# dmlc/difacto

Hardware: AMD Instinct MI355X
Metric: examples/sec (FM SGD worker step, Criteo-shape, V_dim=64) (higher is better)
Workload: dtype f32

## Files before the change

### difacto_amd/csrc/dfh_api.hip

```cpp
#include <algorithm>
#include <chrono>
#include <cstring>
#include <mutex>
#include <new>
#include <thread>

#include <hip/hip_ext.h>
#include <rocprim/rocprim.hpp>

#include "dfh_kernels.hip"
#include "dfh_localize.hip"
#include "dfh_update.hip"
#include "dfh_riders.hip"

using namespace dfh;

namespace dfh {
static thread_local std::string g_err;
void set_error(const std::string& msg) { g_err = msg; }
}

struct dfh_ctx {
  int device = 0;
  hipStream_t stream = nullptr;
// ... 33 lines not shown
  std::vector<hipEvent_t> pool;
  double t_ms[DFH_K_COUNT] = {0};
  uint64_t t_calls[DFH_K_COUNT] = {0};
};

namespace {
struct TimeScope {
  dfh_ctx* c;
  int id;
  hipStream_t st;
  hipEvent_t a = nullptr, b = nullptr;
  static hipEvent_t get(dfh_ctx* c) {
    if (!c->pool.empty()) {
      hipEvent_t e = c->pool.back();
      c->pool.pop_back();
      return e;
    }
    hipEvent_t e = nullptr;
    if (hipEventCreate(&e) != hipSuccess) return nullptr;
    return e;
  }
  TimeScope(dfh_ctx* ctx, int kid, hipStream_t s = nullptr) : c(ctx), id(kid), st(s ? s : ctx->stream) {
    if (kid >= DFH_K_COUNT || !((c->timing >> kid) & 1u)) return;
    a = get(c);
    b = get(c);
    if (a && b) (void)hipEventRecord(a, st);
  }
  ~TimeScope() {
    if (!a || !b) return;
    (void)hipEventRecord(b, st);
    c->spans.push_back({id, a, b});
  }
};
}

struct dfh_table {
  dfh_ctx* ctx = nullptr;
  TableView v{};
  uint64_t hslots = 0;
  uint64_t bytes = 0;
  bool has_aux = true;
  bool auto_grow = false;
  uint64_t rows_bound = 0;
  uint64_t grows = 0;
  uint32_t* d_need = nullptr;
  uint32_t* d_rank = nullptr;
  uint32_t* d_urow = nullptr;
  uint32_t* d_total = nullptr;
  size_t aux_cap = 0;
};

struct dfh_batch {
  dfh_ctx* ctx = nullptr;
  size_t max_rows = 0, max_nnz = 0;
  size_t nrows = 0, nnz = 0;
  bool has_value = false;
  bool has_cnt = false;
  bool localized = false;
  uint64_t* d_raw = nullptr;
  uint32_t* d_offset = nullptr;
  float* d_value = nullptr;
  float* d_label = nullptr;
  void* arena = nullptr;
  void* shared_arena = nullptr;
  size_t arena_bytes = 0;
  uint64_t* o_raw = nullptr;
  uint32_t* o_offset = nullptr;
  float* o_value = nullptr;
  float* o_label = nullptr;
  char* h_stage = nullptr;
  size_t stage_bytes = 0;
  hipEvent_t ev_staged = nullptr;
  bool staged_pending = false;
  double t_prof[6] = {0, 0, 0, 0, 0, 0};
  uint64_t n_prof = 0;
  char* d_stage_view = nullptr;
  bool defer_ready = false;
  uint64_t *d_keys = nullptr, *d_skeys = nullptr;
  uint32_t *d_pos = nullptr, *d_spos = nullptr;
  uint32_t *d_bpos = nullptr;
  uint32_t *d_head = nullptr, *d_uid = nullptr;
  void* d_temp = nullptr;
  size_t temp_bytes = 0;
  uint64_t *d_smp_key = nullptr, *d_spl_key = nullptr, *d_first_key = nullptr, *d_last_key = nullptr;
  uint32_t *d_smp_rank = nullptr, *d_smp_pos = nullptr, *d_spl_pos = nullptr, *d_packed = nullptr, *d_run_off = nullptr,
           *d_bstart = nullptr, *d_btotal = nullptr, *d_nheads = nullptr, *d_lh = nullptr;
  size_t max_tiles = 0;
  int spl_P = 0;
  uint64_t* d_feaids = nullptr;
  float* d_feacnt = nullptr;
  uint32_t *d_col_ptr = nullptr, *d_index = nullptr, *d_s_row = nullptr;
  float* d_s_val = nullptr;
  uint32_t* d_U = nullptr;
  uint2 *d_mid = nullptr, *d_hot = nullptr, *d_few = nullptr;
  SegEnt *d_mid_ent = nullptr, *d_hot_ent = nullptr, *d_few_ent = nullptr;
  SegEnt* d_split_ent = nullptr;
  uint32_t* d_split_ticket = nullptr;
  float* d_split_part = nullptr;
  size_t split_cap = 0;
  int split_sel = 0, split_last = 0;
  bool split_listing = false;
  uint32_t seg_nb = 0;
  uint2* d_uw = nullptr;
  uint32_t *d_urow = nullptr, *d_need = nullptr, *d_rank = nullptr, *d_total = nullptr;
  float *d_pred = nullptr, *d_slope = nullptr, *d_xv = nullptr;
  size_t xv_floats = 0;
  double* d_prog = nullptr;
  float nrows_seen = 0;
  hipEvent_t ev_ready = nullptr, ev_free = nullptr;
  bool ready_pending = false, free_pending = false;
  hipStream_t prep = nullptr;
  bool compute_auc = false;
  uint32_t *d_auc_keys = nullptr, *d_auc_skeys = nullptr, *d_auc_lab = nullptr, *d_auc_slab = nullptr;
  uint32_t* d_auc_part = nullptr;
  uint32_t auc_pending_n = 0;
  bool force_radix = false;
  bool force_sort_fallback = false;
  dfh_table* looked_up = nullptr;
  struct GatherSeg { struct dfh_rowbuf* rb; size_t at, n; };
  std::vector<GatherSeg> gsegs;
  GatherSrc gsrc{};
  bool gather_pending = false, gather_fusable = false, gather_any_value = false, loc_fuse_gather = false;
  const uint32_t *g_rows = nullptr, *g_off = nullptr;
  const float* g_lab = nullptr;
  LocView loc_v{};
  EmitOut loc_o{};
  uint32_t loc_gsort = 0;
  bool loc_big = false;
  int pend_stage = RID_STAGES;
};

namespace {
int flush_pending(dfh_batch* b);
void pend_remove(dfh_ctx* c, dfh_batch* b);
inline hipStream_t prep_of(const dfh_batch* b) {
  const dfh_ctx* c = b->ctx;
  return (c->pipeline && b->prep) ? b->prep : c->stream;
}
void phase_begin(dfh_batch* b) {
  dfh_ctx* c = b->ctx;
  if (b->pend_stage < RID_STAGES) (void)flush_pending(b);
  hipStream_t next = c->pipeline ? c->preps[c->next_prep++ % c->nprep] : nullptr;
  if (next && b->prep && next != b->prep && b->ready_pending) {
    (void)hipStreamWaitEvent(next, b->ev_ready, 0);
  }
  b->prep = next;
}
int prep_begin(dfh_batch* b) {
  dfh_ctx* c = b->ctx;
  if (c->pipeline && !b->prep) phase_begin(b);
  if (c->pipeline && b->free_pending) {
    DFH_HIP(hipStreamWaitEvent(prep_of(b), b->ev_free, 0));
    b->free_pending = false;
  }
  return DFH_OK;
}
int prep_end(dfh_batch* b) {
  dfh_ctx* c = b->ctx;
  if (c->pipeline && !b->defer_ready) {
    DFH_HIP(hipEventRecord(b->ev_ready, prep_of(b)));
    b->ready_pending = true;
  }
  return DFH_OK;
}
int main_begin(dfh_batch* b) {
  dfh_ctx* c = b->ctx;
  if (b->pend_stage < RID_STAGES) {
    int rc = flush_pending(b);
    if (rc) return rc;
// ... 1773 lines not shown
namespace {
struct SharedArena {
  void* base = nullptr;
  int refs = 0;
};
}

static int batch_create_impl(dfh_ctx* c, size_t max_rows, size_t max_nnz, dfh_batch** out, SharedArena* shared, size_t at,
                             size_t* size_only, bool sync) {
  DFH_ARG(c && (out || size_only) && max_rows >= 1 && max_nnz >= 1, "dfh_batch_create: bad argument");
  DFH_ARG(max_nnz < 0xFFFFFFF0ULL && max_rows < 0xFFFFFFF0ULL, "batch too large for 32-bit positions");
  DFH_HIP(hipSetDevice(c->device));
  dfh_batch* b = new (std::nothrow) dfh_batch();
  DFH_ARG(b != nullptr, "out of host memory");
  b->ctx = c;
  b->max_rows = max_rows;
  b->max_nnz = max_nnz;
  const size_t N = max_nnz, B = max_rows;
  size_t sort_bytes = 0, scan_bytes = 0;
  rocprim::radix_sort_pairs(nullptr, sort_bytes, (uint64_t*)nullptr, (uint64_t*)nullptr, (uint32_t*)nullptr,
                            (uint32_t*)nullptr, N, 0, 64, c->stream);
  rocprim::inclusive_scan(nullptr, scan_bytes, (uint32_t*)nullptr, (uint32_t*)nullptr, N, rocprim::plus<uint32_t>(), c->stream);
  size_t auc_bytes = 0;
  rocprim::radix_sort_pairs(nullptr, auc_bytes, (uint32_t*)nullptr, (uint32_t*)nullptr, (uint32_t*)nullptr,
                            (uint32_t*)nullptr, B, 0, 32, c->stream);
  b->temp_bytes = std::max(std::max(sort_bytes, scan_bytes), auc_bytes) + 256;
  char* arena_at = nullptr;
  size_t arena_need = 0;
  bool sizing = true;
#define DFH_ALLOC(ptr, count, type)                                                        \
  do {                                                                                     \
    const size_t bytes__ = (((size_t)(count) * sizeof(type)) + 255) & ~(size_t)255;        \
    if (sizing) {                                                                          \
      arena_need += bytes__;                                                               \
    } else {                                                                               \
      (ptr) = reinterpret_cast<type*>(arena_at);                                           \
      arena_at += bytes__;                                                                 \
    }                                                                                      \
  } while (0)
  for (int pass = 0; pass < 2; ++pass) {
  sizing = pass == 0;
  if (!sizing) {
    if (size_only) {
      *size_only = arena_need;
      delete b;
      return DFH_OK;
    }
    if (shared) {
      b->shared_arena = shared;
      ++shared->refs;
      arena_at = static_cast<char*>(shared->base) + at;
    } else {
      hipError_t e__ = hipMalloc(reinterpret_cast<void**>(&b->arena), arena_need);
      if (e__ != hipSuccess) {
        set_error(std::string("dfh_batch_create: hipMalloc: ") + hipGetErrorString(e__));
        dfh_batch_destroy(b);
        return DFH_ERR_HIP;
      }
      arena_at = static_cast<char*>(b->arena);
    }
  }
  DFH_ALLOC(b->o_raw, N, uint64_t);
  DFH_ALLOC(b->o_offset, B + 1, uint32_t);
  DFH_ALLOC(b->o_value, N, float);
  DFH_ALLOC(b->o_label, B, float);
  b->d_raw = b->o_raw;
  b->d_offset = b->o_offset;
  b->d_value = b->o_value;
  b->d_label = b->o_label;
  DFH_ALLOC(b->d_keys, N, uint64_t);
  DFH_ALLOC(b->d_skeys, N, uint64_t);
  DFH_ALLOC(b->d_pos, N, uint32_t);
  DFH_ALLOC(b->d_spos, N, uint32_t);
  DFH_ALLOC(b->d_bpos, N, uint32_t);
  DFH_ALLOC(b->d_head, N, uint32_t);
  DFH_ALLOC(b->d_uid, N, uint32_t);
  DFH_ALLOC(b->d_temp, b->temp_bytes, char);
  b->max_tiles = (N + LOC_TILE - 1) / LOC_TILE;
  DFH_ALLOC(b->d_spl_key, LOC_BIG_BUCKETS, uint64_t);
  DFH_ALLOC(b->d_spl_pos, LOC_BIG_BUCKETS, uint32_t);
  DFH_ALLOC(b->d_smp_key, LOC_BIG_BUCKETS * LOC_OVERSAMPLE, uint64_t);
  DFH_ALLOC(b->d_smp_pos, LOC_BIG_BUCKETS * LOC_OVERSAMPLE, uint32_t);
  DFH_ALLOC(b->d_smp_rank, LOC_BIG_BUCKETS * LOC_OVERSAMPLE, uint32_t);
  DFH_ALLOC(b->d_first_key, LOC_BIG_BUCKETS, uint64_t);
  DFH_ALLOC(b->d_last_key, LOC_BIG_BUCKETS, uint64_t);
  DFH_ALLOC(b->d_packed, N, uint32_t);
  DFH_ALLOC(b->d_run_off, b->max_tiles * LOC_BIG_BUCKETS, uint32_t);
  DFH_ALLOC(b->d_bstart, LOC_BIG_BUCKETS + 1, uint32_t);
  DFH_ALLOC(b->d_btotal, LOC_XCDS * LOC_BIG_BUCKETS, uint32_t);
  DFH_ALLOC(b->d_nheads, LOC_BIG_BUCKETS, uint32_t);
  DFH_ALLOC(b->d_lh, LOC_BIG_BUCKETS, uint32_t);
  DFH_ALLOC(b->d_feaids, N, uint64_t);
  DFH_ALLOC(b->d_feacnt, N, float);
  DFH_ALLOC(b->d_col_ptr, N + 1, uint32_t);
  DFH_ALLOC(b->d_index, N, uint32_t);
  DFH_ALLOC(b->d_s_row, N, uint32_t);
  DFH_ALLOC(b->d_s_val, N, float);
  DFH_ALLOC(b->d_U, 64, uint32_t);
  DFH_ALLOC(b->d_urow, N, uint32_t);
  DFH_ALLOC(b->d_uw, N, uint2);
  DFH_ALLOC(b->d_mid_ent, N / (BWD_SMALL + 1) + 2 * LOC_BIG_BUCKETS + 16, SegEnt);
  DFH_ALLOC(b->d_hot_ent, N / (BWD_MID + 1) + 2 * LOC_BIG_BUCKETS + 16, SegEnt);
  DFH_ALLOC(b->d_few_ent, N / 2 + 2 * LOC_BIG_BUCKETS + 16, SegEnt);
  b->split_cap = 2 * (N / HOT_SPLIT) + 16;
  DFH_ALLOC(b->d_split_ent, b->split_cap, SegEnt);
  DFH_ALLOC(b->d_split_ticket, b->split_cap, uint32_t);
  DFH_ALLOC(b->d_split_part, b->split_cap * UPD_SPLIT_STRIDE, float);
  DFH_ALLOC(b->d_mid, LOC_BIG_BUCKETS, uint2);
  DFH_ALLOC(b->d_hot, LOC_BIG_BUCKETS, uint2);
  DFH_ALLOC(b->d_few, LOC_BIG_BUCKETS, uint2);
  DFH_ALLOC(b->d_need, N, uint32_t);
  DFH_ALLOC(b->d_rank, N, uint32_t);
  DFH_ALLOC(b->d_pred, B, float);
  DFH_ALLOC(b->d_slope, B, float);
  DFH_ALLOC(b->d_prog, 2 * PROG_SLOTS + 64, double);
  DFH_ALLOC(b->d_auc_keys, B, uint32_t);
  DFH_ALLOC(b->d_auc_skeys, B, uint32_t);
  DFH_ALLOC(b->d_auc_lab, B, uint32_t);
  DFH_ALLOC(b->d_auc_slab, B, uint32_t);
  DFH_ALLOC(b->d_auc_part, AUC_PART_WORDS, uint32_t);
  }
#undef DFH_ALLOC
  b->arena_bytes = arena_need;
  b->d_total = b->d_U + 1;
  const unsigned evf = hipEventDisableTiming | (c->event_flags ? hipEventDisableSystemFence : 0u);
  hipError_t e2 = hipEventCreateWithFlags(&b->ev_ready, evf);
  if (e2 == hipSuccess) e2 = hipEventCreateWithFlags(&b->ev_free, evf);
  if (e2 == hipSuccess) e2 = hipMemsetAsync(b->d_prog, 0, (2 * PROG_SLOTS + 64) * sizeof(double), c->stream);
  if (e2 == hipSuccess) e2 = hipMemsetAsync(b->d_U, 0, 64 * sizeof(uint32_t), c->stream);
  if (e2 == hipSuccess) e2 = hipMemsetAsync(b->d_split_ticket, 0, b->split_cap * sizeof(uint32_t), c->stream);
  if (e2 == hipSuccess) e2 = hipMemsetAsync(b->d_btotal, 0, LOC_XCDS * LOC_BIG_BUCKETS * sizeof(uint32_t), c->stream);
  if (e2 == hipSuccess) e2 = hipMemsetAsync(b->d_urow, 0xFF, N * sizeof(uint32_t), c->stream);
  if (e2 == hipSuccess) e2 = hipMemsetAsync(b->d_uw, 0xFF, N * sizeof(uint2), c->stream);
  if (e2 == hipSuccess && sync) e2 = hipStreamSynchronize(c->stream);
  if (e2 != hipSuccess) {
    set_error(std::string("dfh_batch_create: ") + hipGetErrorString(e2));
    dfh_batch_destroy(b);
    return DFH_ERR_HIP;
  }
  *out = b;
  return DFH_OK;
}

int dfh_batch_create(dfh_ctx* c, size_t max_rows, size_t max_nnz, dfh_batch** out) {
  return batch_create_impl(c, max_rows, max_nnz, out, nullptr, 0, nullptr, true);
}

int dfh_batch_create_many(dfh_ctx* c, int n, size_t max_rows, size_t max_nnz, dfh_batch** out) {
  DFH_ARG(c && out && n >= 1 && n <= 64, "dfh_batch_create_many: 1 <= n <= 64 objects");
  size_t each = 0;
  int rc = batch_create_impl(c, max_rows, max_nnz, nullptr, nullptr, 0, &each, false);
  if (rc) return rc;
  each = (each + 4095) & ~(size_t)4095;
  SharedArena* sa = new (std::nothrow) SharedArena();
  DFH_ARG(sa != nullptr, "out of host memory");
  DFH_HIP(hipSetDevice(c->device));
  if (hipMalloc(&sa->base, each * (size_t)n) != hipSuccess) {
    delete sa;
    set_error("dfh_batch_create_many: hipMalloc failed");
    return DFH_ERR_HIP;
  }
  for (int i = 0; i < n; ++i) out[i] = nullptr;
  sa->refs = 1;
  for (int i = 0; i < n && !rc; ++i) rc = batch_create_impl(c, max_rows, max_nnz, &out[i], sa, each * (size_t)i, nullptr, false);
  if (!rc && hipStreamSynchronize(c->stream) != hipSuccess) {
    set_error("dfh_batch_create_many: hipStreamSynchronize failed");
    rc = DFH_ERR_HIP;
  }
  if (rc) {
    for (int j = 0; j < n; ++j) {
      if (out[j]) dfh_batch_destroy(out[j]);
      out[j] = nullptr;
    }
  }
// ... 583 lines not shown
    rs->period = std::max(1u, per);
  }
}

int localize_impl(dfh_batch* b, uint64_t max_index, dfh_table* probe) {
  dfh_ctx* c = b->ctx;
  DFH_HIP(hipSetDevice(c->device));
  const uint32_t N = (uint32_t)b->nnz;
  if (probe && N) {
    if (int rcr = table_reserve(probe, N)) return rcr;
  }
  {
    int rc = prep_begin(b);
    if (rc) return rc;
  }
  hipStream_t s = prep_of(b);
  b->looked_up = nullptr;
  if (b->pend_stage < RID_STAGES) {
    int rc = flush_pending(b);
    if (rc) return rc;
  }
  if (N == 0) {
    if (b->gather_pending) {
      int rcg = gather_alone(b, s);
      if (rcg) return rcg;
    }
    DFH_HIP(hipMemsetAsync(b->d_U, 0, 64 * sizeof(uint32_t), s));
    DFH_HIP(hipMemsetAsync(b->d_col_ptr, 0, 4, s));
    b->seg_nb = 0;
    b->localized = true;
    return prep_end(b);
  }
  const int g = grid_for_threads(N, c);
  TimeScope* tsp = new TimeScope(c, DFH_K_LOCALIZE, s);
  int P = 0;
  bool cold = true;
  if (b->spl_P > 0 && N / (uint32_t)b->spl_P >= (uint32_t)LOC_MIN_AVG && N / (uint32_t)b->spl_P <= (uint32_t)LOC_MAX_AVG) {
    P = b->spl_P;
    cold = false;
  } else {
#ifndef DFH_LOC_SMALL_AVG
#define DFH_LOC_SMALL_AVG 192
#endif
    const size_t avg_bucket = N <= 65536u ? (size_t)DFH_LOC_SMALL_AVG : (size_t)LOC_AVG_BUCKET;
    const size_t P_want = (N + avg_bucket - 1) / avg_bucket;
    if (P_want <= (size_t)LOC_MAX_BUCKETS) P = (int)std::max<size_t>(1, P_want);
    else if (N / LOC_MAX_BUCKETS <= (uint32_t)LOC_MAX_AVG) P = LOC_MAX_BUCKETS;
    else if (P_want <= (size_t)LOC_BIG_BUCKETS) P = (int)P_want;
    else if (N / LOC_BIG_BUCKETS <= (uint32_t)LOC_MAX_AVG) P = LOC_BIG_BUCKETS;
  }
  b->loc_fuse_gather = b->gather_pending && b->gather_fusable && !cold && P > 0 && P <= LOC_MAX_BUCKETS && !b->force_radix &&
                       !c->single_queue && !getenv("DFH_GATHER_ALONE");
  if (b->gather_pending && !b->loc_fuse_gather) {
    int rcg = gather_alone(b, s);
    if (rcg) return rcg;
  }
  if (P > 0 && !b->force_radix) {
    LocView& v = b->loc_v;
    v.raw = b->d_raw;
    v.n = N;
    v.max_index = max_index;
    v.P = P;
    const bool big = P > LOC_MAX_BUCKETS;
    v.bstride = big ? LOC_BIG_BUCKETS : LOC_MAX_BUCKETS;
    v.ntiles = (int)((N + LOC_TILE - 1) / LOC_TILE);
    v.force_global = b->force_sort_fallback ? 1 : 0;
    v.tb = N > 1 ? std::min(16, __builtin_clz(N - 1)) : 16;
    v.nrows = (uint32_t)b->nrows;
    v.offset = b->d_offset;
    v.rowid = b->d_pos;
    v.smp_key = b->d_smp_key;
    v.smp_pos = b->d_smp_pos;
    v.smp_rank = b->d_smp_rank;
    v.spl_key = b->d_spl_key;
    v.spl_pos = b->d_spl_pos;
    v.packed = b->d_packed;
    v.run_off = b->d_run_off;
    v.btotal = b->d_btotal;
    v.bstart = b->d_bstart;
    v.bkeys = b->d_keys;
    v.bpos = b->d_bpos;
    v.skeys = b->d_skeys;
    v.spos = b->d_spos;
    v.first_key = b->d_first_key;
    v.last_key = b->d_last_key;
    v.nheads = b->d_nheads;
    v.lh = b->d_lh;
    EmitOut& o = b->loc_o;
    o.value = b->has_value ? b->d_value : (const float*)nullptr;
    o.feaids = b->d_feaids;
    o.col_ptr = b->d_col_ptr;
    o.index = b->d_index;
    o.s_row = b->d_s_row;
    o.s_val = b->d_s_val;
    o.d_U = b->d_U;
    o.sl.mid = b->d_mid;
    o.sl.mid_ent = b->d_mid_ent;
    o.sl.hot = b->d_hot;
    o.sl.hot_ent = b->d_hot_ent;
    o.sl.few = b->d_few;
    o.sl.few_ent = b->d_few_ent;
    v.split_n = b->d_U + 2;
    b->loc_big = big;
#ifndef DFH_LOC_GRID_CAP
#define DFH_LOC_GRID_CAP 1024
#endif
    b->loc_gsort = (unsigned)std::min<int>(P, big ? LOC_BIG_BUCKETS : DFH_LOC_GRID_CAP);
    if (cold && P > 1) {
      const uint32_t S = (uint32_t)P * LOC_OVERSAMPLE;
      const uint32_t nt = (S + 255) / 256;
      hipLaunchKernelGGL(k_ss_sample, dim3(nt), dim3(256), 0, s, v);
      hipLaunchKernelGGL(k_ss_rank, dim3(nt * nt), dim3(256), 0, s, v);
      hipLaunchKernelGGL(k_loc_splitters, dim3(nt), dim3(256), 0, s, v);
    }
    if (c->single_queue && !cold && !big && !probe) {
      b->pend_stage = 0;
      c->pend.push_back(b);
    } else {
      for (int st = 0; st < RID_STAGES; ++st) {
        launch_loc_stage(b, st, s, probe);
        if (st == RID_COUNT && b->loc_fuse_gather) {
          int rcg = gather_queued(b, s);
          b->loc_fuse_gather = false;
          if (rcg) return rcg;
        }
      }
    }
    b->spl_P = P;
    b->seg_nb = (uint32_t)P;
  } else {
    hipLaunchKernelGGL(k_rdx_keys, dim3(g), dim3(256), 0, s, b->d_raw, N, max_index, b->d_keys, b->d_pos);
    size_t tb = b->temp_bytes;
    DFH_HIP(rocprim::radix_sort_pairs(b->d_temp, tb, b->d_keys, b->d_skeys, b->d_pos, b->d_spos, (size_t)N, 0, 64, s));
    hipLaunchKernelGGL(k_rdx_heads, dim3(g), dim3(256), 0, s, b->d_skeys, N, b->d_head);
    tb = b->temp_bytes;
    DFH_HIP(rocprim::inclusive_scan(b->d_temp, tb, b->d_head, b->d_uid, (size_t)N, rocprim::plus<uint32_t>(), s));
    hipLaunchKernelGGL(k_rdx_emit, dim3(g), dim3(256), 0, s, b->d_skeys, b->d_spos, b->d_head, b->d_uid, N, (uint32_t)b->nrows,
                       b->d_offset, b->has_value ? b->d_value : (const float*)nullptr, b->d_feaids, b->d_col_ptr, b->d_index,
                       b->d_s_row, b->d_s_val, b->d_U);
    hipLaunchKernelGGL(k_seg_lists_reset, dim3(1), dim3(64), 0, s, b->d_mid, b->d_hot, b->d_few, b->d_U + 2);
    hipLaunchKernelGGL(k_seg_lists, dim3((unsigned)std::max<size_t>(1, std::min<size_t>((N + 1023) / 1024, 256))), dim3(1024), 0, s,
                       b->d_col_ptr, b->d_U, b->d_mid, b->d_hot, b->d_few, b->d_mid_ent, b->d_hot_ent, b->d_few_ent);
    b->seg_nb = 1;
    if (probe)
      hipLaunchKernelGGL(k_lookup, dim3(grid_for_threads(b->nnz, c)), dim3(256), 0, s, probe->v, b->d_feaids, b->d_U, 0u, b->d_urow,
                         (const float*)nullptr, b->d_col_ptr, 0, (uint32_t*)nullptr, 0, (uint2*)nullptr, AucFin{nullptr, 0u, nullptr});
  }
  delete tsp;
  DFH_HIP(hipGetLastError());
  b->localized = true;
  b->has_cnt = false;
  if (probe) b->looked_up = probe;
  return prep_end(b);
}
}


namespace {
struct DescribedIn {
  size_t nrows, nnz;
  int nseg;
  dfh_rowbuf* const* bufs;
  const size_t* seg_rows;
  bool any_value;
  const uint32_t *v_rows, *v_off;
  const float* v_lab;
  const uint32_t* v_tile;
  bool fusable;
  const uint32_t* v_base;
};
// ... 656 lines not shown
```

### difacto_amd/csrc/dfh_localize.hip

```cpp
#ifndef DFH_LOCALIZE_HIP_
#define DFH_LOCALIZE_HIP_
#include "dfh_internal.h"

namespace dfh {

constexpr int LOC_OVERSAMPLE = 8;
constexpr int LOC_MAX_BUCKETS = 1024;
constexpr int LOC_BIG_BUCKETS = 4096;
constexpr int LOC_AVG_BUCKET = 384;
constexpr int LOC_MIN_AVG = 48;
constexpr int LOC_MAX_AVG = 700;
constexpr int LOC_LDS_CAP = 1024;
#ifndef DFH_LOC_TILE
#define DFH_LOC_TILE 2048
#endif
#ifndef DFH_LOC_TILE_THREADS
#define DFH_LOC_TILE_THREADS 1024
#endif
constexpr int LOC_TILE = DFH_LOC_TILE;
constexpr int LOC_TILE_THREADS = DFH_LOC_TILE_THREADS;
constexpr int LOC_PER_THREAD = LOC_TILE / LOC_TILE_THREADS;
constexpr int LOC_SORT_THREADS = 256;
constexpr int LOC_EMIT_THREADS = 256;

struct LocView {
  const uint64_t* raw;
  uint32_t n;
  uint64_t max_index;
  int P;
  int bstride;
  int ntiles;
  int force_global;
  int tb;
  uint32_t nrows;
  const uint32_t* offset;
  const uint32_t* rowid;
  uint64_t* smp_key;
  uint32_t* smp_pos;
  uint32_t* smp_rank;
  uint64_t* spl_key;
  uint32_t* spl_pos;
  uint32_t* packed;
  uint32_t* run_off;
  uint32_t* btotal;
  uint32_t* bstart;
  uint64_t* bkeys;
  uint32_t* bpos;
  uint64_t* skeys;
  uint32_t* spos;
  uint64_t* first_key;
  uint64_t* last_key;
  uint32_t* nheads;
  uint32_t* lh;
  uint32_t* split_n;
};

struct SegListsOut {
  uint2* mid;
  SegEnt* mid_ent;
  uint2* hot;
  SegEnt* hot_ent;
  uint2* few;
  SegEnt* few_ent;
};

__device__ __forceinline__ uint64_t make_key(uint64_t id, uint64_t max_index) {
  const uint64_t m = (max_index == ~0ULL) ? (id == ~0ULL ? 0ULL : id) : id % max_index;
  return reverse_bytes(m);
}

constexpr int LOC_XCDS = 8;

__device__ __forceinline__ bool comp_less(uint64_t ka, uint32_t pa, uint64_t kb, uint32_t pb) {
  return ka < kb || (ka == kb && pa < pb);
}

template <bool MAX>
__device__ __forceinline__ uint32_t wave_inclusive(uint32_t x) {
#define DFH_DPP_STEP(ctrl, row_mask)                                                                      \
  {                                                                                                       \
    const uint32_t y = (uint32_t)__builtin_amdgcn_update_dpp(0, (int)x, ctrl, row_mask, 0xf, false);    \
    x = MAX ? max(x, y) : x + y;                                                                          \
  }
  DFH_DPP_STEP(0x111, 0xf)
  DFH_DPP_STEP(0x112, 0xf)
  DFH_DPP_STEP(0x114, 0xf)
  DFH_DPP_STEP(0x118, 0xf)
  DFH_DPP_STEP(0x142, 0xa)
  DFH_DPP_STEP(0x143, 0xc)
#undef DFH_DPP_STEP
  return x;
}

template <bool MAX, int NWAVES>
__device__ __forceinline__ uint32_t block_exclusive(uint32_t val, uint32_t* wtot , uint32_t* total) {
  static_assert(NWAVES <= 64, "one lane per wave");
  const int lane = (int)(threadIdx.x & 63);
  const int w = __builtin_amdgcn_readfirstlane((int)(threadIdx.x >> 6));
  const uint32_t s = wave_inclusive<MAX>(val);
  __syncthreads();
  if (lane == 63) wtot[w] = s;
  __syncthreads();
  const uint32_t x = wave_inclusive<MAX>(lane < NWAVES ? wtot[lane] : 0u);
  const uint32_t before = w ? (uint32_t)__builtin_amdgcn_readlane((int)x, w - 1) : 0u;
  if (total) *total = (uint32_t)__builtin_amdgcn_readlane((int)x, NWAVES - 1);
  const uint32_t prev = (uint32_t)__builtin_amdgcn_update_dpp(0, (int)s, 0x138, 0xf, 0xf, false);
  return MAX ? max(before, prev) : before + prev;
}
template <int NWAVES>
__device__ __forceinline__ uint32_t block_exclusive_scan(uint32_t val, uint32_t* wsum , uint32_t* total) {
  return block_exclusive<false, NWAVES>(val, wsum, total);
}
template <int NWAVES>
__device__ __forceinline__ uint32_t block_exclusive_max(uint32_t val, uint32_t* wmax , uint32_t* total) {
  return block_exclusive<true, NWAVES>(val, wmax, total);
}

__device__ __forceinline__ uint32_t ss_sample_pos(uint32_t t, uint32_t stride, uint32_t n) {
  const uint32_t j = (uint32_t)(splitmix64(t) >> 33) % stride;
  return min(t * stride + j, n - 1);
}

__global__ void __launch_bounds__(256) k_ss_sample(LocView v) {
  const uint32_t S = (uint32_t)v.P * LOC_OVERSAMPLE;
  const uint32_t stride = max(1u, v.n / S);
  for (uint32_t t = blockIdx.x * blockDim.x + threadIdx.x; t < S; t += gridDim.x * blockDim.x) {
    const uint32_t i = ss_sample_pos(t, stride, v.n);
    v.smp_key[t] = make_key(v.raw[i], v.max_index);
    v.smp_pos[t] = i << v.tb;
    v.smp_rank[t] = 0;
  }
}

__global__ void __launch_bounds__(256) k_ss_rank(LocView v) {
  __shared__ uint64_t ck[256];
  __shared__ uint32_t cp[256];
  const uint32_t S = (uint32_t)v.P * LOC_OVERSAMPLE;
  const uint32_t ntile = (S + 255) / 256;
  const uint32_t ti = blockIdx.x / ntile, tj = blockIdx.x % ntile;
  const uint32_t col = tj * 256 + threadIdx.x;
  ck[threadIdx.x] = col < S ? v.smp_key[col] : ~0ULL;
  cp[threadIdx.x] = col < S ? v.smp_pos[col] : ~0u;
  const uint32_t row = ti * 256 + threadIdx.x;
  const uint64_t mk = row < S ? v.smp_key[row] : 0;
  const uint32_t mp = row < S ? v.smp_pos[row] : 0;
  __syncthreads();
  const uint32_t lim = min(256u, S - tj * 256);
  uint32_t rank = 0;
#pragma unroll 8
  for (uint32_t j = 0; j < lim; ++j) {
    const bool less = comp_less(ck[j], cp[j], mk, mp) || (ck[j] == mk && cp[j] == mp && tj * 256 + j < row);
    rank += less ? 1u : 0u;
  }
  if (row < S && rank) atomicAdd(&v.smp_rank[row], rank);
}

__global__ void __launch_bounds__(256) k_loc_splitters(LocView v) {
  const uint32_t S = (uint32_t)v.P * LOC_OVERSAMPLE;
  for (uint32_t t = blockIdx.x * blockDim.x + threadIdx.x; t < S; t += gridDim.x * blockDim.x) {
    const uint32_t r = v.smp_rank[t];
    if (r > 0 && r % LOC_OVERSAMPLE == 0) {
      v.spl_key[r / LOC_OVERSAMPLE - 1] = v.smp_key[t];
      v.spl_pos[r / LOC_OVERSAMPLE - 1] = v.smp_pos[t];
    }
  }
}

constexpr int LOC_GATHER_ROWS = 1024;
constexpr int LOC_GATHER_SEGS = 4;
struct GatherSrc {
  int nseg;
  uint32_t seg_row0[LOC_GATHER_SEGS + 1];
  const uint32_t* src_off[LOC_GATHER_SEGS];
  const uint64_t* src_idx[LOC_GATHER_SEGS];
  const float* src_val[LOC_GATHER_SEGS];
  const uint32_t* h_rows;
  const uint32_t* h_off;
  const float* h_lab;
  const uint32_t* h_tile_row;
  uint64_t* dst_raw;
  float* dst_val;
  uint32_t* dst_off;
  float* dst_lab;
};
constexpr size_t loc_gather_smem() { return (size_t)(LOC_GATHER_ROWS + 1) * 4 + 4 + (size_t)LOC_GATHER_ROWS * 8; }
template <typename T>
__device__ __forceinline__ T loc_sel(const T (&a)[LOC_GATHER_SEGS], uint32_t sg) {
  T r = a[0];
#pragma unroll
  for (int x = 1; x < LOC_GATHER_SEGS; ++x) r = sg == (uint32_t)x ? a[x] : r;
  return r;
}

template <int MAXB>
constexpr size_t loc_count_smem() { return (size_t)MAXB * 16; }
template <int MAXB, int THREADS>
constexpr size_t loc_scatter_smem() { return (size_t)MAXB * 4 + (THREADS / 64) * 4; }
constexpr size_t loc_sort_smem() { return (size_t)LOC_LDS_CAP * 24 + 2 * (LOC_SORT_THREADS / 64) * 4; }
constexpr size_t loc_emit_smem() { return (2 * (LOC_EMIT_THREADS / 64) + 4) * 4; }

template <int MAXB, int THREADS, bool GATHER = false>
__device__ __forceinline__ void loc_count_block(const LocView& v, const uint32_t bid, const uint32_t nblk, char* smem,
                                                const GatherSrc* gp = nullptr) {
  constexpr int PER = LOC_TILE / THREADS;
  static_assert(PER * THREADS == LOC_TILE, "a tile is a whole number of elements per thread");
  uint64_t* sk = reinterpret_cast<uint64_t*>(smem);
  uint32_t* sp = reinterpret_cast<uint32_t*>(smem + (size_t)MAXB * 8);
  uint32_t* hist = sp + MAXB;
  const int P = v.P;
  for (int b = threadIdx.x; b < P; b += THREADS) {
    hist[b] = 0;
    sk[b] = b < P - 1 ? v.spl_key[b] : ~0ULL;
    sp[b] = b < P - 1 ? v.spl_pos[b] : ~0u;
  }
  const uint32_t base = bid * LOC_TILE;
  if (bid == 0 && threadIdx.x == 0 && v.split_n) *v.split_n = 0u;
  uint64_t key[PER];
  if (GATHER) {
    const GatherSrc& g = *gp;
    uint32_t* roff = reinterpret_cast<uint32_t*>(smem + loc_count_smem<MAXB>());
    uint64_t* rsrc = reinterpret_cast<uint64_t*>(roff + LOC_GATHER_ROWS + 2);
    const uint32_t row0 = g.h_tile_row[bid], row1 = g.h_tile_row[bid + 1];
    const uint32_t nr = min(row1, v.nrows - 1u) - row0 + 1u;
    for (uint32_t q = threadIdx.x; q <= nr; q += THREADS) roff[q] = g.h_off[row0 + q];
    for (uint32_t q = threadIdx.x; q < nr; q += THREADS) {
      const uint32_t r = row0 + q;
      uint32_t sg = 0;
#pragma unroll
      for (int x = 1; x < LOC_GATHER_SEGS; ++x) sg += (x < g.nseg && r >= g.seg_row0[x]) ? 1u : 0u;
      rsrc[q] = ((uint64_t)loc_sel(g.src_off, sg)[g.h_rows[r]] << 2) | sg;
    }
    __syncthreads();
#pragma unroll
    for (int e = 0; e < PER; ++e) {
      const uint32_t i = base + e * THREADS + threadIdx.x;
      key[e] = ~0ULL;
      if (i < v.n) {
        uint32_t lo = 0, hi = nr - 1u;
        while (lo < hi) {
          const uint32_t mid = (lo + hi + 1u) >> 1;
          if (roff[mid] <= i) lo = mid; else hi = mid - 1u;
        }
        const uint64_t sw = rsrc[lo];
        const uint32_t sg = (uint32_t)(sw & 3u);
        const size_t at = (size_t)(sw >> 2) + (i - roff[lo]);
        const uint64_t id = loc_sel(g.src_idx, sg)[at];
        g.dst_raw[i] = id;
        if (g.dst_val) {
          const float* sv = loc_sel(g.src_val, sg);
          g.dst_val[i] = sv ? sv[at] : 1.0f;
        }
        key[e] = make_key(id, v.max_index);
      }
    }
  } else {
#pragma unroll
    for (int e = 0; e < PER; ++e) {
      const uint32_t i = base + e * THREADS + threadIdx.x;
      key[e] = i < v.n ? make_key(v.raw[i], v.max_index) : ~0ULL;
    }
  }
  {
    uint32_t* __restrict__ rowid = const_cast<uint32_t*>(v.rowid);
    const uint32_t* __restrict__ offset = GATHER ? gp->h_off : v.offset;
    const uint32_t rpb = (v.nrows + nblk - 1) / nblk;
    const uint32_t r0 = bid * rpb, r1 = min(v.nrows, r0 + rpb);
    for (uint32_t r = r0 + threadIdx.x; r < r1; r += THREADS) {
      const uint32_t b0 = offset[r], e = offset[r + 1];
      if (GATHER) {
        gp->dst_off[r] = b0;
        gp->dst_lab[r] = gp->h_lab[r];
        if (r + 1 == v.nrows) gp->dst_off[r + 1] = e;
      }
      for (uint32_t j = b0; j < e; ++j) rowid[j] = r;
    }
  }
  __syncthreads();
  int lo[PER], hi[PER];
#pragma unroll
  for (int e = 0; e < PER; ++e) { lo[e] = 0; hi[e] = P - 1; }
  for (int step = P; step > 1; step = (step + 1) >> 1) {
#pragma unroll
// ... 266 lines not shown
    for (uint32_t j = 0; j < lim; ++j) rank += comp_less(xk[c0 + j], xp[c0 + j], mk, mp) ? 1u : 0u;
    if (valid) {
      yk[c0 + rank] = mk;
      yp[c0 + rank] = mp;
    }
  }
  __syncthreads();
  uint64_t* srck = yk; uint32_t* srcp = yp;
  uint64_t* dstk = xk; uint32_t* dstp = xp;
  for (uint32_t L = 64; L < n; L <<= 1) {
    for (uint32_t idx = threadIdx.x; idx < n; idx += blockDim.x) {
      const uint64_t mk = srck[idx];
      const uint32_t mp = srcp[idx];
      const uint32_t r = idx / L;
      const uint32_t pair_base = (r & ~1u) * L;
      const uint32_t sib = (r ^ 1u) * L;
      uint32_t lo = min(sib, n), hi = min(sib + L, n);
      const uint32_t sib_beg = lo;
      while (lo < hi) {
        const uint32_t mid = (lo + hi) >> 1;
        if (comp_less(srck[mid], srcp[mid], mk, mp)) lo = mid + 1; else hi = mid;
      }
      const uint32_t dst = pair_base + (idx - r * L) + (lo - sib_beg);
      dstk[dst] = mk;
      dstp[dst] = mp;
    }
    __syncthreads();
    uint64_t* tk = srck; srck = dstk; dstk = tk;
    uint32_t* tp = srcp; srcp = dstp; dstp = tp;
  }
  if (srck != yk) {
    for (uint32_t t = threadIdx.x; t < n; t += blockDim.x) {
      yk[t] = srck[t];
      yp[t] = srcp[t];
    }
  }
  __syncthreads();
}

struct BucketSummary {
  uint32_t nheads, lh;
  uint64_t first_key, last_key;
};
template <bool WRITE>
__device__ __forceinline__ BucketSummary loc_bucket_summary(const uint64_t* sk, const uint32_t* sp, uint32_t n, uint64_t* ok,
                                                            uint32_t* op, uint32_t (*red)[LOC_SORT_THREADS / 64]) {
  uint32_t cnt = 0, last = 0;
  uint32_t t0 = threadIdx.x;
  asm volatile("" : "+v"(t0));
  for (uint32_t t = t0; t < n; t += LOC_SORT_THREADS) {
    const uint64_t k = sk[t];
    if (WRITE) {
      ok[t] = k;
      op[t] = sp[t];
    }
    if (t + 1 < n && sk[t + 1] != k) {
      ++cnt;
      last = t + 1;
    }
  }
  cnt = (uint32_t)__builtin_amdgcn_readlane((int)wave_inclusive<false>(cnt), 63);
  last = (uint32_t)__builtin_amdgcn_readlane((int)wave_inclusive<true>(last), 63);
  if ((threadIdx.x & 63) == 0) {
    red[0][threadIdx.x >> 6] = cnt;
    red[1][threadIdx.x >> 6] = last;
  }
  __syncthreads();
  BucketSummary r;
  r.nheads = 1;
  r.lh = 0;
  r.first_key = 0;
  r.last_key = 0;
  if (threadIdx.x == 0) {
    for (int w = 0; w < LOC_SORT_THREADS / 64; ++w) {
      r.nheads += red[0][w];
      r.lh = max(r.lh, red[1][w]);
    }
    r.first_key = sk[0];
    r.last_key = sk[n - 1];
  }
  return r;
}

__device__ __forceinline__ void loc_sort_block(const LocView& v, const uint32_t bid, const uint32_t nblk, char* smem) {
  uint64_t* ak = reinterpret_cast<uint64_t*>(smem);
  uint64_t* bk = ak + LOC_LDS_CAP;
  uint32_t* ap = reinterpret_cast<uint32_t*>(bk + LOC_LDS_CAP);
  uint32_t* bp = ap + LOC_LDS_CAP;
  uint32_t (*red)[LOC_SORT_THREADS / 64] = reinterpret_cast<uint32_t (*)[LOC_SORT_THREADS / 64]>(bp + LOC_LDS_CAP);
  for (uint32_t b = bid; b < (uint32_t)v.P; b += nblk) {
    __syncthreads();
    const uint32_t beg = v.bstart[b], end = v.bstart[b + 1];
    const uint32_t n = end - beg;
    if (threadIdx.x < LOC_XCDS) v.btotal[threadIdx.x * v.bstride + b] = 0;
    if (n == 0) {
      if (threadIdx.x == 0) {
        v.nheads[b] = 0;
        v.lh[b] = 0;
        v.first_key[b] = 0;
        v.last_key[b] = 0;
      }
      continue;
    }
    BucketSummary sm;
    if (n <= LOC_LDS_CAP && !v.force_global) {
      const bool in_a = loc_sort_bucket_lds(v, beg, n, ak, ap, bk, bp);
      sm = loc_bucket_summary<true>(in_a ? ak : bk, in_a ? ap : bp, n, v.skeys + beg, v.spos + beg, red);
    } else {
      loc_sort_bucket_global(v, beg, n);
      sm = loc_bucket_summary<false>(v.skeys + beg, v.spos + beg, n, nullptr, nullptr, red);
    }
    if (threadIdx.x == 0) {
      v.nheads[b] = sm.nheads;
      v.lh[b] = sm.lh;
      v.first_key[b] = sm.first_key;
      v.last_key[b] = sm.last_key;
    }
  }
}
__global__ void __launch_bounds__(LOC_SORT_THREADS) k_loc_sort(LocView v) {
  extern __shared__ __attribute__((aligned(16))) char smem[];
  loc_sort_block(v, blockIdx.x, gridDim.x, smem);
}

template <int NW, bool PROBE>
__device__ __forceinline__ void loc_emit_bucket(const LocView& v, uint32_t b, uint32_t beg, uint32_t n, const uint64_t* sk,
                                                const uint32_t* sp, uint32_t cont, uint32_t ubase, uint32_t carry1,
                                                const float* __restrict__ value,
                                                uint64_t* __restrict__ feaids, uint32_t* __restrict__ col_ptr,
                                                uint32_t* __restrict__ index, uint32_t* __restrict__ s_row,
                                                float* __restrict__ s_val, uint32_t* __restrict__ d_U, const SegListsOut& sl,
                                                uint32_t* wsum, uint32_t* wmax, uint32_t* n_mid, uint32_t* n_hot,
                                                uint32_t* n_few, const TableView& tab, uint32_t* __restrict__ urow) {
  const uint32_t P = (uint32_t)v.P;
  const uint32_t moff = beg / (BWD_SMALL + 1) + 2 * b, hoff = beg / (BWD_MID + 1) + 2 * b, foff = beg / 2 + 2 * b;
  uint32_t run_heads = 0, run_max1 = carry1;
  for (uint32_t base = 0; base < n; base += blockDim.x) {
    const uint32_t t = base + threadIdx.x;
    const uint32_t i = beg + t;
    const bool valid = t < n;
    uint64_t key = 0;
    uint32_t tag = 0;
    bool head = false;
    if (valid) {
      key = sk[t];
      tag = sp[t];
      head = t == 0 ? !cont : key != sk[t - 1];
    }
    const uint32_t pos = tag >> v.tb;
    uint32_t nh, mx;
    const uint32_t ex = block_exclusive_scan<NW>(head ? 1u : 0u, wsum, &nh);
    const uint32_t pm = block_exclusive_max<NW>(head ? i + 1 : 0u, wmax, &mx);
    if (valid) {
      const uint32_t incl = run_heads + ex + (head ? 1u : 0u);
      const uint32_t uid = ubase + incl - 1;
      const uint32_t prev1 = max(run_max1, pm);
      if (head) {
        feaids[uid] = key;
        col_ptr[uid] = i;
        if (PROBE) urow[uid] = find_or_insert(tab, key);
        if (prev1) {
          const uint32_t len = i - (prev1 - 1);
          const SegEnt e = make_uint4(uid - 1, prev1 - 1, i, 0u);
          if (len > BWD_MID) sl.hot_ent[hoff + atomicAdd(n_hot, 1u)] = e;
          else if (len > BWD_SMALL) sl.mid_ent[moff + atomicAdd(n_mid, 1u)] = e;
          else if (len > 1) sl.few_ent[foff + atomicAdd(n_few, 1u)] = e;
        }
      }
      index[pos] = uid;
      uint32_t row = tag & ((1u << v.tb) - 1u);
      {
        const uint32_t step = 1u << v.tb;
        uint32_t lo = 0, hi = v.nrows > row ? (v.nrows - 1u - row) >> v.tb : 0u;
        while (lo < hi) {
          const uint32_t mid = (lo + hi + 1u) >> 1;
          if (v.offset[row + mid * step] <= pos) lo = mid; else hi = mid - 1u;
        }
        row += lo * step;
      }
      s_row[i] = row;
      if (value) s_val[i] = value[pos];
      if (i == v.n - 1) {
        *d_U = uid + 1;
        col_ptr[uid + 1] = v.n;
        const uint32_t lbeg = head ? i : prev1 - 1, len = v.n - lbeg;
        const SegEnt e = make_uint4(uid, lbeg, v.n, 0u);
        if (len > BWD_MID) sl.hot_ent[hoff + atomicAdd(n_hot, 1u)] = e;
        else if (len > BWD_SMALL) sl.mid_ent[moff + atomicAdd(n_mid, 1u)] = e;
        else if (len > 1) sl.few_ent[foff + atomicAdd(n_few, 1u)] = e;
      }
    }
    run_heads += nh;
    run_max1 = max(run_max1, mx);
  }
  if (P > 1) {
    const uint64_t N = v.n;
    const uint64_t m0 = max((uint64_t)beg * P / N + ((uint64_t)beg * P % N ? 1u : 0u), (uint64_t)1);
    const uint64_t e1 = (uint64_t)(beg + n) * P;
    const uint64_t m1 = min(e1 / N + (e1 % N ? 1u : 0u), (uint64_t)P);
    for (uint64_t m = m0 + threadIdx.x; m < m1; m += blockDim.x) {
      const uint32_t i = (uint32_t)(m * N / P);
      if ((i * (uint64_t)P + N - 1) / N == m) {
        v.spl_key[m - 1] = sk[i - beg];
        v.spl_pos[m - 1] = sp[i - beg];
      }
    }
  }
  __syncthreads();
  if (threadIdx.x == 0) {
    sl.mid[b] = make_uint2(*n_mid, moff);
    sl.hot[b] = make_uint2(*n_hot, hoff);
    sl.few[b] = make_uint2(*n_few, foff);
  }
}

struct EmitOut {
  const float* value;
  uint64_t* feaids;
  uint32_t* col_ptr;
  uint32_t* index;
  uint32_t* s_row;
  float* s_val;
  uint32_t* d_U;
  SegListsOut sl;
};

template <bool PROBE>
__device__ __forceinline__ void loc_emit_block(const LocView& v, const EmitOut& o, const TableView& tab, uint32_t* __restrict__ urow,
                                               const uint32_t bid, const uint32_t nblk, char* smem) {
  constexpr int NW = LOC_EMIT_THREADS / 64;
  uint32_t* wsum = reinterpret_cast<uint32_t*>(smem);
  uint32_t* wmax = wsum + NW;
  uint32_t& sh_cont = wmax[NW];
  uint32_t& n_mid = wmax[NW + 1];
  uint32_t& n_hot = wmax[NW + 2];
  uint32_t& n_few = wmax[NW + 3];
  const SegListsOut& sl = o.sl;
  const uint32_t P = (uint32_t)v.P;
  for (uint32_t b = bid; b < P; b += nblk) {
    __syncthreads();
    const uint32_t beg = v.bstart[b], end = v.bstart[b + 1];
    const uint32_t n = end - beg;
    if (threadIdx.x == 0) {
      n_mid = 0;
      n_hot = 0;
      n_few = 0;
      if (n == 0) {
        sl.mid[b] = make_uint2(0u, 0u);
        sl.hot[b] = make_uint2(0u, 0u);
        sl.few[b] = make_uint2(0u, 0u);
      }
    }
    if (n == 0) continue;
    uint32_t part = 0, carry1 = 0;
    for (uint32_t q0 = threadIdx.x; q0 <= b; q0 += LOC_EMIT_THREADS) {
      const uint32_t bq = v.bstart[q0], nq = v.bstart[q0 + 1] - bq;
      if (nq == 0) continue;
      int p = (int)q0 - 1;
      while (p >= 0 && v.bstart[p + 1] == v.bstart[p]) --p;
      const uint32_t c = (p >= 0 && v.first_key[q0] == v.last_key[p]) ? 1u : 0u;
      if (q0 == b) {
        sh_cont = c;
      } else {
        part += v.nheads[q0] - c;
        const uint32_t l = v.lh[q0];
        if (l > 0) carry1 = max(carry1, bq + l + 1);
        else if (!c) carry1 = max(carry1, bq + 1);
      }
    }
    uint32_t ubase, carry_all;
    block_exclusive_scan<NW>(part, wsum, &ubase);
    block_exclusive_max<NW>(carry1, wmax, &carry_all);
    __syncthreads();
    loc_emit_bucket<NW, PROBE>(v, b, beg, n, v.skeys + beg, v.spos + beg, sh_cont, ubase, carry_all, o.value, o.feaids, o.col_ptr,
                               o.index, o.s_row, o.s_val, o.d_U, sl, wsum, wmax, &n_mid, &n_hot, &n_few, tab, urow);
  }
}

template <bool PROBE>
__global__ void __launch_bounds__(LOC_EMIT_THREADS) k_loc_emit(LocView v, EmitOut o, TableView tab, uint32_t* __restrict__ urow) {
  __shared__ __attribute__((aligned(16))) char smem[loc_emit_smem()];
  loc_emit_block<PROBE>(v, o, tab, urow, blockIdx.x, gridDim.x, smem);
}

}
#endif
```

Measured before the change: 88.42 million.

## Pack per-bucket summaries into 32-byte records and fuse emit block scans

```diff
diff --git a/difacto_amd/csrc/dfh_api.hip b/difacto_amd/csrc/dfh_api.hip
--- a/difacto_amd/csrc/dfh_api.hip
+++ b/difacto_amd/csrc/dfh_api.hip
@@ -139,9 +139,10 @@
   uint32_t *d_head = nullptr, *d_uid = nullptr;
   void* d_temp = nullptr;
   size_t temp_bytes = 0;
-  uint64_t *d_smp_key = nullptr, *d_spl_key = nullptr, *d_first_key = nullptr, *d_last_key = nullptr;
+  uint64_t *d_smp_key = nullptr, *d_spl_key = nullptr;
+  BucketRec* d_brec = nullptr;
   uint32_t *d_smp_rank = nullptr, *d_smp_pos = nullptr, *d_spl_pos = nullptr, *d_packed = nullptr, *d_run_off = nullptr,
-           *d_bstart = nullptr, *d_btotal = nullptr, *d_nheads = nullptr, *d_lh = nullptr;
+           *d_bstart = nullptr, *d_btotal = nullptr;
   size_t max_tiles = 0;
   int spl_P = 0;
   uint64_t* d_feaids = nullptr;
@@ -2081,14 +2082,11 @@
   DFH_ALLOC(b->d_smp_key, LOC_BIG_BUCKETS * LOC_OVERSAMPLE, uint64_t);
   DFH_ALLOC(b->d_smp_pos, LOC_BIG_BUCKETS * LOC_OVERSAMPLE, uint32_t);
   DFH_ALLOC(b->d_smp_rank, LOC_BIG_BUCKETS * LOC_OVERSAMPLE, uint32_t);
-  DFH_ALLOC(b->d_first_key, LOC_BIG_BUCKETS, uint64_t);
-  DFH_ALLOC(b->d_last_key, LOC_BIG_BUCKETS, uint64_t);
+  DFH_ALLOC(b->d_brec, LOC_BIG_BUCKETS, BucketRec);
   DFH_ALLOC(b->d_packed, N, uint32_t);
   DFH_ALLOC(b->d_run_off, b->max_tiles * LOC_BIG_BUCKETS, uint32_t);
   DFH_ALLOC(b->d_bstart, LOC_BIG_BUCKETS + 1, uint32_t);
   DFH_ALLOC(b->d_btotal, LOC_XCDS * LOC_BIG_BUCKETS, uint32_t);
-  DFH_ALLOC(b->d_nheads, LOC_BIG_BUCKETS, uint32_t);
-  DFH_ALLOC(b->d_lh, LOC_BIG_BUCKETS, uint32_t);
   DFH_ALLOC(b->d_feaids, N, uint64_t);
   DFH_ALLOC(b->d_feacnt, N, float);
   DFH_ALLOC(b->d_col_ptr, N + 1, uint32_t);
@@ -2838,10 +2836,7 @@
     v.bpos = b->d_bpos;
     v.skeys = b->d_skeys;
     v.spos = b->d_spos;
-    v.first_key = b->d_first_key;
-    v.last_key = b->d_last_key;
-    v.nheads = b->d_nheads;
-    v.lh = b->d_lh;
+    v.brec = b->d_brec;
     EmitOut& o = b->loc_o;
     o.value = b->has_value ? b->d_value : (const float*)nullptr;
     o.feaids = b->d_feaids;
diff --git a/difacto_amd/csrc/dfh_localize.hip b/difacto_amd/csrc/dfh_localize.hip
--- a/difacto_amd/csrc/dfh_localize.hip
+++ b/difacto_amd/csrc/dfh_localize.hip
@@ -22,6 +22,16 @@
 constexpr int LOC_PER_THREAD = LOC_TILE / LOC_TILE_THREADS;
 constexpr int LOC_SORT_THREADS = 256;
 constexpr int LOC_EMIT_THREADS = 256;
+
+struct __attribute__((aligned(32))) BucketRec {
+  uint64_t first_key;
+  uint32_t nheads;
+  uint32_t lh1;
+  uint32_t beg;
+  uint32_t count;
+  uint64_t last_key;
+};
+static_assert(sizeof(BucketRec) == 32, "one record is two 16-byte halves");
 
 struct LocView {
   const uint64_t* raw;
@@ -48,10 +58,7 @@
   uint32_t* bpos;
   uint64_t* skeys;
   uint32_t* spos;
-  uint64_t* first_key;
-  uint64_t* last_key;
-  uint32_t* nheads;
-  uint32_t* lh;
+  BucketRec* brec;
   uint32_t* split_n;
 };
 
@@ -75,19 +82,19 @@
   return ka < kb || (ka == kb && pa < pb);
 }
 
-template <bool MAX>
+template <bool MAX, int WIDTH = 64>
 __device__ __forceinline__ uint32_t wave_inclusive(uint32_t x) {
 #define DFH_DPP_STEP(ctrl, row_mask)                                                                      \
   {                                                                                                       \
     const uint32_t y = (uint32_t)__builtin_amdgcn_update_dpp(0, (int)x, ctrl, row_mask, 0xf, false);    \
     x = MAX ? max(x, y) : x + y;                                                                          \
   }
-  DFH_DPP_STEP(0x111, 0xf)
-  DFH_DPP_STEP(0x112, 0xf)
-  DFH_DPP_STEP(0x114, 0xf)
-  DFH_DPP_STEP(0x118, 0xf)
-  DFH_DPP_STEP(0x142, 0xa)
-  DFH_DPP_STEP(0x143, 0xc)
+  if constexpr (WIDTH > 1) DFH_DPP_STEP(0x111, 0xf)
+  if constexpr (WIDTH > 2) DFH_DPP_STEP(0x112, 0xf)
+  if constexpr (WIDTH > 4) DFH_DPP_STEP(0x114, 0xf)
+  if constexpr (WIDTH > 8) DFH_DPP_STEP(0x118, 0xf)
+  if constexpr (WIDTH > 16) DFH_DPP_STEP(0x142, 0xa)
+  if constexpr (WIDTH > 32) DFH_DPP_STEP(0x143, 0xc)
 #undef DFH_DPP_STEP
   return x;
 }
@@ -111,9 +118,26 @@
 __device__ __forceinline__ uint32_t block_exclusive_scan(uint32_t val, uint32_t* wsum , uint32_t* total) {
   return block_exclusive<false, NWAVES>(val, wsum, total);
 }
+
 template <int NWAVES>
-__device__ __forceinline__ uint32_t block_exclusive_max(uint32_t val, uint32_t* wmax , uint32_t* total) {
-  return block_exclusive<true, NWAVES>(val, wmax, total);
+__device__ __forceinline__ void block_exclusive_sum_max(uint32_t a, uint32_t m, uint2* wtot ,
+                                                        uint32_t& ex_sum, uint32_t& ex_max, uint32_t& tot_sum, uint32_t& tot_max) {
+  static_assert(NWAVES <= 64, "one lane per wave");
+  const int lane = (int)(threadIdx.x & 63);
+  const int w = __builtin_amdgcn_readfirstlane((int)(threadIdx.x >> 6));
+  const uint32_t sa = wave_inclusive<false>(a);
+  const uint32_t sm = wave_inclusive<true>(m);
+  if (lane == 63) wtot[w] = make_uint2(sa, sm);
+  __syncthreads();
+  const uint2 t = wtot[min(lane, NWAVES - 1)];
+  const uint32_t xa = wave_inclusive<false, NWAVES>(lane < NWAVES ? t.x : 0u);
+  const uint32_t xm = wave_inclusive<true, NWAVES>(lane < NWAVES ? t.y : 0u);
+  const uint32_t ba = w ? (uint32_t)__builtin_amdgcn_readlane((int)xa, w - 1) : 0u;
+  const uint32_t bm = w ? (uint32_t)__builtin_amdgcn_readlane((int)xm, w - 1) : 0u;
+  tot_sum = (uint32_t)__builtin_amdgcn_readlane((int)xa, NWAVES - 1);
+  tot_max = (uint32_t)__builtin_amdgcn_readlane((int)xm, NWAVES - 1);
+  ex_sum = ba + (uint32_t)__builtin_amdgcn_update_dpp(0, (int)sa, 0x138, 0xf, 0xf, false);
+  ex_max = max(bm, (uint32_t)__builtin_amdgcn_update_dpp(0, (int)sm, 0x138, 0xf, 0xf, false));
 }
 
 __device__ __forceinline__ uint32_t ss_sample_pos(uint32_t t, uint32_t stride, uint32_t n) {
@@ -197,7 +221,7 @@
 template <int MAXB, int THREADS>
 constexpr size_t loc_scatter_smem() { return (size_t)MAXB * 4 + (THREADS / 64) * 4; }
 constexpr size_t loc_sort_smem() { return (size_t)LOC_LDS_CAP * 24 + 2 * (LOC_SORT_THREADS / 64) * 4; }
-constexpr size_t loc_emit_smem() { return (2 * (LOC_EMIT_THREADS / 64) + 4) * 4; }
+constexpr size_t loc_emit_smem() { return (2 * 2 * (LOC_EMIT_THREADS / 64) + 4) * 4; }
 
 template <int MAXB, int THREADS, bool GATHER = false>
 __device__ __forceinline__ void loc_count_block(const LocView& v, const uint32_t bid, const uint32_t nblk, char* smem,
@@ -630,6 +654,12 @@
   return r;
 }
 
+__device__ __forceinline__ void loc_write_rec(BucketRec* r, const BucketSummary& sm, uint32_t beg, uint32_t n) {
+  uint4* h = reinterpret_cast<uint4*>(r);
+  h[0] = make_uint4((uint32_t)sm.first_key, (uint32_t)(sm.first_key >> 32), sm.nheads, n ? beg + sm.lh + 1u : 0u);
+  h[1] = make_uint4(beg, n, (uint32_t)sm.last_key, (uint32_t)(sm.last_key >> 32));
+}
+
 __device__ __forceinline__ void loc_sort_block(const LocView& v, const uint32_t bid, const uint32_t nblk, char* smem) {
   uint64_t* ak = reinterpret_cast<uint64_t*>(smem);
   uint64_t* bk = ak + LOC_LDS_CAP;
@@ -642,12 +672,7 @@
     const uint32_t n = end - beg;
     if (threadIdx.x < LOC_XCDS) v.btotal[threadIdx.x * v.bstride + b] = 0;
     if (n == 0) {
-      if (threadIdx.x == 0) {
-        v.nheads[b] = 0;
-        v.lh[b] = 0;
-        v.first_key[b] = 0;
-        v.last_key[b] = 0;
-      }
+      if (threadIdx.x == 0) loc_write_rec(v.brec + b, BucketSummary{0u, 0u, 0, 0}, beg, 0u);
       continue;
     }
     BucketSummary sm;
@@ -658,12 +683,7 @@
       loc_sort_bucket_global(v, beg, n);
       sm = loc_bucket_summary<false>(v.skeys + beg, v.spos + beg, n, nullptr, nullptr, red);
     }
-    if (threadIdx.x == 0) {
-      v.nheads[b] = sm.nheads;
-      v.lh[b] = sm.lh;
-      v.first_key[b] = sm.first_key;
-      v.last_key[b] = sm.last_key;
-    }
+    if (threadIdx.x == 0) loc_write_rec(v.brec + b, sm, beg, n);
   }
 }
 __global__ void __launch_bounds__(LOC_SORT_THREADS) k_loc_sort(LocView v) {
@@ -678,12 +698,14 @@
                                                 uint64_t* __restrict__ feaids, uint32_t* __restrict__ col_ptr,
                                                 uint32_t* __restrict__ index, uint32_t* __restrict__ s_row,
                                                 float* __restrict__ s_val, uint32_t* __restrict__ d_U, const SegListsOut& sl,
-                                                uint32_t* wsum, uint32_t* wmax, uint32_t* n_mid, uint32_t* n_hot,
+                                                uint2* wtot, uint32_t* n_mid, uint32_t* n_hot,
                                                 uint32_t* n_few, const TableView& tab, uint32_t* __restrict__ urow) {
   const uint32_t P = (uint32_t)v.P;
   const uint32_t moff = beg / (BWD_SMALL + 1) + 2 * b, hoff = beg / (BWD_MID + 1) + 2 * b, foff = beg / 2 + 2 * b;
   uint32_t run_heads = 0, run_max1 = carry1;
-  for (uint32_t base = 0; base < n; base += blockDim.x) {
+  const bool two_rows = ((v.nrows - 1u) >> v.tb) <= 1u;
+  uint32_t area = NW;
+  for (uint32_t base = 0; base < n; base += blockDim.x, area ^= NW) {
     const uint32_t t = base + threadIdx.x;
     const uint32_t i = beg + t;
     const bool valid = t < n;
@@ -696,9 +718,8 @@
       head = t == 0 ? !cont : key != sk[t - 1];
     }
     const uint32_t pos = tag >> v.tb;
-    uint32_t nh, mx;
-    const uint32_t ex = block_exclusive_scan<NW>(head ? 1u : 0u, wsum, &nh);
-    const uint32_t pm = block_exclusive_max<NW>(head ? i + 1 : 0u, wmax, &mx);
+    uint32_t ex, pm, nh, mx;
+    block_exclusive_sum_max<NW>(head ? 1u : 0u, head ? i + 1 : 0u, wtot + area, ex, pm, nh, mx);
     if (valid) {
       const uint32_t incl = run_heads + ex + (head ? 1u : 0u);
       const uint32_t uid = ubase + incl - 1;
@@ -717,8 +738,12 @@
       }
       index[pos] = uid;
       uint32_t row = tag & ((1u << v.tb) - 1u);
-      {
-        const uint32_t step = 1u << v.tb;
+      const uint32_t step = 1u << v.tb;
+      if (two_rows) {
+        const uint32_t r1 = row + step;
+        const uint32_t o1 = v.offset[min(r1, v.nrows)];
+        row = (r1 < v.nrows && o1 <= pos) ? r1 : row;
+      } else {
         uint32_t lo = 0, hi = v.nrows > row ? (v.nrows - 1u - row) >> v.tb : 0u;
         while (lo < hi) {
           const uint32_t mid = (lo + hi + 1u) >> 1;
@@ -730,7 +755,9 @@
       if (value) s_val[i] = value[pos];
       if (i == v.n - 1) {
         *d_U = uid + 1;
-        col_ptr[uid + 1] = v.n;
+        uint32_t n_all = v.n;
+        asm volatile("" : "+s"(n_all));
+        col_ptr[uid + 1] = n_all;
         const uint32_t lbeg = head ? i : prev1 - 1, len = v.n - lbeg;
         const SegEnt e = make_uint4(uid, lbeg, v.n, 0u);
         if (len > BWD_MID) sl.hot_ent[hoff + atomicAdd(n_hot, 1u)] = e;
@@ -777,14 +804,18 @@
 __device__ __forceinline__ void loc_emit_block(const LocView& v, const EmitOut& o, const TableView& tab, uint32_t* __restrict__ urow,
                                                const uint32_t bid, const uint32_t nblk, char* smem) {
   constexpr int NW = LOC_EMIT_THREADS / 64;
-  uint32_t* wsum = reinterpret_cast<uint32_t*>(smem);
-  uint32_t* wmax = wsum + NW;
-  uint32_t& sh_cont = wmax[NW];
-  uint32_t& n_mid = wmax[NW + 1];
-  uint32_t& n_hot = wmax[NW + 2];
-  uint32_t& n_few = wmax[NW + 3];
+  constexpr int REC = 2;
+  uint2* wtot = reinterpret_cast<uint2*>(smem);
+  uint32_t* word = reinterpret_cast<uint32_t*>(wtot + 2 * NW);
+  uint32_t& sh_cont = word[0];
+  uint32_t& n_mid = word[1];
+  uint32_t& n_hot = word[2];
+  uint32_t& n_few = word[3];
   const SegListsOut& sl = o.sl;
   const uint32_t P = (uint32_t)v.P;
+  const BucketRec* __restrict__ rec = v.brec;
+  const char* __restrict__ recb = reinterpret_cast<const char*>(v.brec);
+  typedef uint3 __attribute__((aligned(4))) RecTail;
   for (uint32_t b = bid; b < P; b += nblk) {
     __syncthreads();
     const uint32_t beg = v.bstart[b], end = v.bstart[b + 1];
@@ -801,27 +832,56 @@
     }
     if (n == 0) continue;
     uint32_t part = 0, carry1 = 0;
-    for (uint32_t q0 = threadIdx.x; q0 <= b; q0 += LOC_EMIT_THREADS) {
-      const uint32_t bq = v.bstart[q0], nq = v.bstart[q0 + 1] - bq;
-      if (nq == 0) continue;
-      int p = (int)q0 - 1;
-      while (p >= 0 && v.bstart[p + 1] == v.bstart[p]) --p;
-      const uint32_t c = (p >= 0 && v.first_key[q0] == v.last_key[p]) ? 1u : 0u;
-      if (q0 == b) {
-        sh_cont = c;
-      } else {
-        part += v.nheads[q0] - c;
-        const uint32_t l = v.lh[q0];
-        if (l > 0) carry1 = max(carry1, bq + l + 1);
-        else if (!c) carry1 = max(carry1, bq + 1);
-      }
-    }
-    uint32_t ubase, carry_all;
-    block_exclusive_scan<NW>(part, wsum, &ubase);
-    block_exclusive_max<NW>(carry1, wmax, &carry_all);
-    __syncthreads();
+    for (uint32_t q0 = threadIdx.x; q0 <= b; q0 += REC * LOC_EMIT_THREADS) {
+      uint4 cur[REC];
+      uint3 prv[REC];
+#pragma unroll
+      for (int r = 0; r < REC; ++r) {
+        const uint32_t q = min(q0 + r * LOC_EMIT_THREADS, b), p = max(q, 1u) - 1u;
+        cur[r] = *reinterpret_cast<const uint4*>(recb + (q << 5));
+        prv[r] = *reinterpret_cast<const RecTail*>(recb + ((p << 5) + (uint32_t)offsetof(BucketRec, count)));
+      }
+#pragma unroll
+      for (int r = 0; r < REC; ++r)
+        asm volatile("" : "+v"(cur[r].x), "+v"(cur[r].y), "+v"(cur[r].z), "+v"(cur[r].w), "+v"(prv[r].x), "+v"(prv[r].y), "+v"(prv[r].z));
+      uint64_t fk[REC], pk[REC];
+      uint32_t nh[REC], l1[REC], pc[REC];
+#pragma unroll
+      for (int r = 0; r < REC; ++r) {
+        fk[r] = ((uint64_t)cur[r].y << 32) | cur[r].x;
+        nh[r] = cur[r].z;
+        l1[r] = cur[r].w;
+        pc[r] = prv[r].x;
+        pk[r] = ((uint64_t)prv[r].z << 32) | prv[r].y;
+      }
+#pragma unroll
+      for (int r = 0; r < REC; ++r) {
+        const uint32_t q = q0 + r * LOC_EMIT_THREADS;
+        if (q > b || nh[r] == 0) continue;
+        uint32_t c = 0;
+        if (q > 0) {
+          uint64_t lk = pk[r];
+          bool any = pc[r] != 0;
+          if (!any) {
+            int p = (int)q - 2;
+            while (p >= 0 && rec[p].count == 0) --p;
+            any = p >= 0;
+            if (any) lk = rec[p].last_key;
+          }
+          c = (any && fk[r] == lk) ? 1u : 0u;
+        }
+        if (q == b) {
+          sh_cont = c;
+        } else {
+          part += nh[r] - c;
+          if (nh[r] > 1 || !c) carry1 = max(carry1, l1[r]);
+        }
+      }
+    }
+    uint32_t ubase, carry_all, ex_unused, pm_unused;
+    block_exclusive_sum_max<NW>(part, carry1, wtot, ex_unused, pm_unused, ubase, carry_all);
     loc_emit_bucket<NW, PROBE>(v, b, beg, n, v.skeys + beg, v.spos + beg, sh_cont, ubase, carry_all, o.value, o.feaids, o.col_ptr,
-                               o.index, o.s_row, o.s_val, o.d_U, sl, wsum, wmax, &n_mid, &n_hot, &n_few, tab, urow);
+                               o.index, o.s_row, o.s_val, o.d_U, sl, wtot, &n_mid, &n_hot, &n_few, tab, urow);
   }
 }
 
```

Measured after the change: 88.61 million (median of 6 runs). About the same (+0.2%).
